# google/nerfactor

Measured on AMD Instinct MI355X. Metric: rays/sec (NeRF coarse+fine render, 64+128 samples/ray), higher is better.
Workload: dtype bf16

## Files before the change

### include/nfx.h

```cpp
#ifndef NFX_H_
#define NFX_H_

#include <stddef.h>
#include <stdint.h>

#ifdef __cplusplus
extern "C" {
#endif

#if defined(__GNUC__)
#define NFX_API __attribute__((visibility("default")))
#else
#define NFX_API
#endif

#define NFX_OK 0
#define NFX_EINVAL (-1)
#define NFX_EALIGN (-2)
#define NFX_EHIP (-3)
#define NFX_ENOSUP (-4)

#define NFX_PREC_BF16 0
#define NFX_PREC_FP32 1
#define NFX_PREC_FP32_NATIVE 2
// ... 187 lines not shown
#define NFX_LOSS_BLEND_A 1
#define NFX_LOSS_BLEND_B 2
#define NFX_LOSS_ACCUM_A 4
#define NFX_LOSS_ACCUM_B 8
typedef struct nfx_loss_term {
    const float *a, *b;
    float *ga, *gb;
    int d;
    float w;
    int kind;
    int flags;
} nfx_loss_term;
NFX_API int nfx_pair_loss_fwd(const nfx_loss_term *terms, int n_terms, const float *dev_alpha, float bg, int64_t n,
                      float *dev_loss, void *stream);
NFX_API int nfx_pair_loss_bwd(const nfx_loss_term *terms, int n_terms, const float *dev_alpha, float bg, int64_t n,
                      const float *dev_dloss, void *stream);


NFX_API int nfx_nerf_sigma_fwd(const float *dev_rayo, const float *dev_rayd, const float *dev_z, int64_t n_rays,
                       int n_samples, const void *dev_geom_blob, int prec, float *dev_sigma, void *stream);

NFX_API size_t nfx_nerf_geom_packed_bytes(int prec);
NFX_API int nfx_nerf_pack_geom_weights(const float *const kernels[12], const float *const biases[12], int prec,
                               void *blob, size_t blob_bytes);
NFX_API int nfx_nerf_sigma_grad(const float *dev_rayo, const float *dev_rayd, const float *dev_z, int64_t n_rays,
                        int n_samples, const void *dev_geom_blob, int prec, float *dev_normal_sigma,
                        void *stream);

NFX_API size_t nfx_nerf_sigma_grad_workspace_bytes(int64_t n_rays, int n_samples);
NFX_API int nfx_nerf_sigma_grad_rows(const float *dev_rayo, const float *dev_rayd, const float *dev_z, int64_t n_rays,
                             int n_samples, const void *dev_geom_blob, int prec, float *dev_normal_sigma,
                             void *dev_workspace, size_t workspace_bytes, void *stream);

NFX_API int nfx_nerf_refine_select(const float *dev_rgbs, const float *dev_z, const float *dev_rayd, int64_t n_rays,
                           int n_samples, float t_min, float a_lo, float a_hi, float sigma_margin, int dilate,
                           int *dev_list, int *dev_count, void *stream);
NFX_API int nfx_nerf_sigma_refine(const float *dev_rayo, const float *dev_rayd, const float *dev_z, int64_t n_rays,
                          int n_samples, const void *dev_geom_blob_fp32, const int *dev_list, const int *dev_count,
                          float *dev_rgbs, void *stream);

#define NFX_OCCGRID_MAX_RES 1024
#define NFX_OCCGRID_MAX_PROBES (1ll << 30)
NFX_API int nfx_nerf_sigma_fwd_list(const float *dev_rayo, const float *dev_rayd, const float *dev_z, int64_t n_rays,
                            int n_samples, const void *dev_geom_blob, int prec, const int *dev_list,
                            const int *dev_count, float *dev_sigma, void *stream);
NFX_API size_t nfx_occgrid_workspace_bytes(int64_t n_rays, int n_samples);
NFX_API int nfx_occgrid_select(const float *dev_rayo, const float *dev_rayd, const float *dev_z, int64_t n_rays,
                       int n_samples, const uint32_t *dev_bits, int res, const float *box, const float *bbox,
                       float *dev_sigma, void *dev_workspace, size_t workspace_bytes, void *stream);
NFX_API int nfx_occgrid_bake(const float *dev_probe_sigma, int res, int probes, float margin, int dilate,
                     uint32_t *dev_bits, uint32_t *dev_workspace, void *stream);


NFX_API int nfx_selftest_mfma_bf16(const float *dev_a, const float *dev_b, float *dev_d, void *stream);
NFX_API int nfx_mlp_generic_split_hilo(void *dev_blob, int d_in, int n_layers, const int *widths, const int *skip_input,
                                       int train, void *stream);
NFX_API size_t nfx_mlp_generic_packed_bytes(int d_in, int n_layers, const int *widths, const int *skip_input, int prec);
NFX_API int nfx_mlp_generic_pack(const float *const *kernels, const float *const *biases, int d_in, int n_layers,
                                 const int *widths, const int *skip_input, int prec, void *blob, size_t blob_bytes);
NFX_API int nfx_mlp_generic_fwd(const float *dev_x, int64_t n, int ld_x, int d_in, int n_layers, const int *widths,
                                const int *acts, const int *skip_input, const void *dev_blob, int prec, float *dev_y,
                                int ld_y, int col0, void *stream);
NFX_API size_t nfx_mlp_generic_train_packed_bytes(int d_in, int n_layers, const int *widths, const int *skip_input,
                                                  int prec);
NFX_API int nfx_mlp_generic_pack_train(const float *const *kernels, const float *const *biases, int d_in, int n_layers,
                                       const int *widths, const int *skip_input, int prec, void *blob,
// ... 21 lines not shown
```

### nerfactor_amd/_capi.py

```python
import ctypes
import os

import torch

_HERE = os.path.dirname(os.path.abspath(__file__))
LIB_PATH = os.path.join(_HERE, 'libnfx.so')
if os.environ.get('NFX_LIB_PATH'):
    LIB_PATH = os.environ['NFX_LIB_PATH']

PREC_BF16, PREC_FP32, PREC_FP32_NATIVE = 0, 1, 2
ACT_NONE, ACT_RELU, ACT_SIGMOID, ACT_SOFTPLUS = 0, 1, 2, 3
IN_XYZ, IN_XYZ_LDIR, IN_Z_RUSINK = 0, 1, 2

if not os.path.exists(LIB_PATH):
    raise ImportError(
        "%s not found: build it with `python -m nerfactor_amd.build` (or __graft_entry__.build()); "
        "nerfactor_amd has no fallback path." % LIB_PATH)

lib = ctypes.CDLL(LIB_PATH)

_p = ctypes.c_void_p
_i = ctypes.c_int
_i64 = ctypes.c_int64
_f = ctypes.c_float
# ... 35 lines not shown
    'nfx_composite_bwd': (_i, [_p, _p, _p, _p, _i64, _i, _i, _p, _p, _p]),
    'nfx_nerf_train_packed_bytes': (_sz, [_i]),
    'nfx_nerf_pack_train_weights': (_i, [_pp, _pp, _i, _p, _sz]),
    'nfx_nerf_bwd_workspace_bytes': (_sz, [_i64, _i]),
    'nfx_nerf_mlp_bwd': (_i, [_p, _p, _p, _i64, _i, _p, _i, _p, _p, _sz, _pp, _pp, _p]),
    'nfx_brdf_train_packed_bytes': (_sz, []),
    'nfx_brdf_pack_train_weights': (_i, [_pp, _pp, _i, _i, _p, _sz]),
    'nfx_brdf_spec_bwd_workspace_bytes': (_sz, [_i, _i64]),
    'nfx_brdf_spec_bwd': (_i, [_p, _p, _p, _p, _i, _p, _i, _p, _i, _i64, _p, _p, _p, _p, _sz, _p]),
    'nfx_brdf_spec_bwd_list_bytes': (_sz, [_i64, _i]),
    'nfx_brdf_spec_bwd_rows': (_i, [_p, _p, _p, _p, _i, _p, _i, _p, _i, _i64, _p, _p, _p, _p, _sz, _p, _sz, _p]),
    'nfx_brdf_rows_fwd': (_i, [_p, _i, _p, _i64, _i, _p, _i, _p, _p]),
    'nfx_brdf_rows_bwd_workspace_bytes': (_sz, [_i, _i64, _i]),
    'nfx_brdf_rows_bwd': (_i, [_p, _i, _p, _i64, _i, _p, _i, _p, _p, _sz, _p, _pp, _pp, _p]),
    'nfx_shade_bwd_workspace_bytes': (_sz, [_i]),
    'nfx_shade_bwd': (_i, [_p, _p, _p, _p, _p, _p, _f, _f, _p, _p, _p, _p, _i64, _i, _i, _p, _p, _p, _p, _p, _p,
                           _p, _p, _sz, _p]),
    'nfx_l2_normalize_rows': (_i, [_p, _p, _i64, _i, _f, _p]),
    'nfx_l2_normalize_rows_bwd': (_i, [_p, _p, _p, _i64, _i, _f, _p]),
    'nfx_light_smoothness': (_i, [_p, _i, _i, _f, _f, _p, _p, _p]),
    'nfx_pair_loss_fwd': (_i, [_p, _i, _p, _f, _i64, _p, _p]),
    'nfx_pair_loss_bwd': (_i, [_p, _i, _p, _f, _i64, _p, _p]),
    'nfx_pack_gather': (_i, [_p, _p, _i64, _p, _p]),
    'nfx_amsgrad_step': (_i, [_p, _p, _p, _p, _p, _i64, _f, _f, _f, _f, _i64, _p]),
    'nfx_amsgrad_step_size': (_f, [_f, _f, _f, _i64]),
    'nfx_amsgrad_step_dev': (_i, [_p, _p, _p, _p, _p, _i64, _p, _f, _f, _f, _p]),
    'nfx_nerf_sigma_fwd': (_i, [_p, _p, _p, _i64, _i, _p, _i, _p, _p]),
    'nfx_lvis_fwd_rows': (_i, [_p, _p, _i64, _f, _p, _i, _p, _i, _p, _sz, _p, _p, _p, _p]),
    'nfx_zero_rows': (_i, [_p, _p, _i64, _i, _p]),
    'nfx_shade_fwd_rows': (_i, [_p, _p, _p, _p, _p, _p, _f, _f, _p, _p, _p, _p, _p, _i64, _i, _i, _i, _p, _p]),
    'nfx_shade_olat_fwd_rows': (_i, [_p, _p, _p, _p, _p, _p, _f, _f, _p, _p, _p, _p, _f, _f, _i64, _i, _i, _p, _p, _p, _p]),
    'nfx_nerf_refine_select': (_i, [_p, _p, _p, _i64, _i, _f, _f, _f, _f, _i, _p, _p, _p]),
    'nfx_nerf_sigma_refine': (_i, [_p, _p, _p, _i64, _i, _p, _p, _p, _p, _p]),
    'nfx_nerf_sigma_fwd_list': (_i, [_p, _p, _p, _i64, _i, _p, _i, _p, _p, _p, _p]),
    'nfx_occgrid_workspace_bytes': (_sz, [_i64, _i]),
    'nfx_occgrid_select': (_i, [_p, _p, _p, _i64, _i, _p, _i, _p, _p, _p, _p, _sz, _p]),
    'nfx_occgrid_bake': (_i, [_p, _i, _i, _f, _i, _p, _p, _p]),
    'nfx_nerf_geom_packed_bytes': (_sz, [_i]),
    'nfx_nerf_pack_geom_weights': (_i, [_pp, _pp, _i, _p, _sz]),
    'nfx_nerf_sigma_grad': (_i, [_p, _p, _p, _i64, _i, _p, _i, _p, _p]),
    'nfx_nerf_sigma_grad_workspace_bytes': (_sz, [_i64, _i]),
    'nfx_nerf_sigma_grad_rows': (_i, [_p, _p, _p, _i64, _i, _p, _i, _p, _p, _sz, _p]),
    'nfx_selftest_mfma_bf16': (_i, [_p, _p, _p, _p]),
    'nfx_selftest_sincos': (_i, [_p, _i64, _i, _p, _p]),
    'nfx_selftest_tr16': (_i, [_p, _p, _p, _i, _p]),
    'nfx_mlp_generic_packed_bytes': (_sz, [_i, _i, _p, _p, _i]),
    'nfx_mlp_generic_pack': (_i, [_pp, _pp, _i, _i, _p, _p, _i, _p, _sz]),
    'nfx_mlp_generic_fwd': (_i, [_p, _i64, _i, _i, _i, _p, _p, _p, _p, _i, _p, _i, _i, _p]),
    'nfx_mlp_generic_train_packed_bytes': (_sz, [_i, _i, _p, _p, _i]),
    'nfx_mlp_generic_pack_train': (_i, [_pp, _pp, _i, _i, _p, _p, _i, _p, _sz]),
    'nfx_mlp_generic_bwd_workspace_bytes': (_sz, [_i64, _i, _i, _p, _p, _i]),
    'nfx_mlp_generic_split_hilo': (_i, [_p, _i, _i, _p, _p, _i, _p]),
    'nfx_brdf_rows_geom_fwd': (_i, [_p, _p, _p, _p, _i, _p, _i, _i64, _i, _p, _i, _p, _p]),
    'nfx_brdf_rows_geom_bwd': (_i, [_p, _p, _p, _i, _p, _i, _i64, _i, _p, _i, _p, _p, _p]),
    'nfx_embed_bwd': (_i, [_p, _i64, _i, _i, _p, _i, _i, _p, _p]),
    'nfx_mlp_generic_bwd': (_i, [_p, _i64, _i, _i, _i, _p, _p, _p, _p, _i, _p, _i, _i, _p, _i, _pp, _pp, _p, _sz, _p]),
    'nfx_embed': (_i, [_p, _p, _p, _i64, _i, _i, _i, _i, _p, _i, _i, _p]),
}

for _name, (_res, _args) in SIGNATURES.items():
    _fn = getattr(lib, _name)
    _fn.restype = _res
    _fn.argtypes = _args


class NfxError(RuntimeError):
# ... 59 lines not shown
```

### nerfactor_amd/csrc/capi_geom.cpp

```cpp
#include <hip/hip_runtime.h>
#include <math.h>
#include <string.h>

#include <vector>

#include "../../include/nfx.h"
#include "nerf_geom_layout.hpp"
#include "pack.hpp"

int nfx_fail(int code, const char* fmt, ...);
int nfx_hip_result(int e, const char* what);
extern "C" int nfx_option_int(const char* name, int dflt);

#define REQUIRE(cond, ...) \
    do {                   \
        if (!(cond)) return nfx_fail(NFX_EINVAL, __VA_ARGS__); \
    } while (0)
#define ALIGNED(p, a) ((((uintptr_t)(p)) & ((a)-1)) == 0)

extern "C" {
int nfx_launch_nerf_sigma_geo(const float*, const float*, const float*, long long, int, const void*, float*, int,
                              hipStream_t);
int nfx_launch_nerf_sigma_grad(const float*, const float*, const float*, long long, int, const void*, float*, int,
                               hipStream_t);
int nfx_launch_refine_select(const float*, const float*, const float*, long long, int, float, float, float, float, int, int*, int*,
                             hipStream_t);
int nfx_launch_nerf_sigma_v6(const float*, const float*, const float*, long long, int, const void*, float*, int, hipStream_t);
int nfx_launch_nerf_sigma_grad_list(const float*, const float*, const float*, long long, int, const void*, float*, const int*,
                                    const int*, int, hipStream_t);
int nfx_launch_nerf_sigma_grad_x3_list(const float*, const float*, const float*, long long, int, const void*, float*,
                                       const int*, const int*, int, hipStream_t);
int nfx_launch_select_density(const float*, long long, float*, void*, hipStream_t);
size_t nfx_nerf_bwd_list_bytes(long long n_pts);
int nfx_launch_nerf_sigma_x3_list(const float*, const float*, const float*, long long, int, const void*, float*, const int*,
                                  const int*, int, hipStream_t);
int nfx_launch_nerf_sigma_x3(const float*, const float*, const float*, long long, int, const void*, float*, int,
                             hipStream_t);
int nfx_launch_nerf_sigma_grad_x3(const float*, const float*, const float*, long long, int, const void*, float*, int,
                                  hipStream_t);
int nfx_launch_nerf_sigma_v6_list(const float*, const float*, const float*, long long, int, const void*, float*, const int*,
                                  const int*, int, hipStream_t);
int nfx_launch_nerf_sigma_x3_list_flat(const float*, const float*, const float*, long long, int, const void*, float*,
                                       const int*, const int*, int, hipStream_t);
size_t nfx_occgrid_list_bytes(long long n_pts);
int nfx_launch_occgrid_select(const float*, const float*, const float*, long long, int, const uint32_t*, int, const float*,
                              const float*, float*, void*, hipStream_t);
int nfx_launch_occgrid_bake(const float*, int, int, float, int, uint32_t*, uint32_t*, hipStream_t);

size_t nfx_nerf_geom_packed_bytes(int prec) {
    using namespace nfx::nerf;
    if (prec == NFX_PREC_BF16) return (size_t)kGeoBlobBytes;
    if (prec == NFX_PREC_FP32) return 2 * (size_t)kGeoWeightBytes + kGeoFloats * sizeof(float);
    return 0;
}
}

static int pack_geom_half(const float* const kernels[12], const float* const biases[12], uint8_t* w0, float* fl) {
    using namespace nfx;
    using namespace nfx::pack;
    std::vector<uint8_t> fwd(nfx_nerf_packed_bytes(NFX_PREC_BF16));
    int rc = nfx_nerf_pack_weights(kernels, biases, NFX_PREC_BF16, fwd.data(), fwd.size());
    if (rc) return rc;
    const size_t enc_bytes = (size_t)nerf::chunk_frag_offset(64) * 1024;
    memcpy(w0, fwd.data(), enc_bytes);
    memcpy(w0 + enc_bytes, fwd.data() + (size_t)nerf::chunk_frag_offset(72) * 1024, 16 * 1024);
    uint8_t* w = w0 + enc_bytes + 16 * 1024;
    std::vector<float> sink(256);
    const Seg hid256{kHidden, 256, 0, nullptr};
    auto hidden_t = [](const float* k) {
        std::vector<float> t((size_t)256 * 256);
        for (int r = 0; r < 256; ++r)
            for (int c = 0; c < 256; ++c) t[(size_t)c * 256 + r] = k[(size_t)r * 256 + c];
        return t;
    };
// ... 57 lines not shown
        }
        lo_ptr[i] = lo[i].data();
    }
    std::vector<float> sink(nerf::kGeoFloats);
    int rc = pack_geom_half(kernels, biases, w0, reinterpret_cast<float*>(w0 + 2 * (size_t)nerf::kGeoWeightBytes));
    if (rc) return rc;
    return pack_geom_half(lo_ptr, biases, w0 + nerf::kGeoWeightBytes, sink.data());
}

static int launch_sigma_bf16(const float* rayo, const float* rayd, const float* z, long long n_pts, int n_samples,
                             const void* blob, float* sigma, hipStream_t st) {
    const int blocks = nfx_option_int("nerf_blocks", 256);
    if (nfx_option_int("sigma_variant", 1) != 0)
        return nfx_launch_nerf_sigma_v6(rayo, rayd, z, n_pts, n_samples, blob, sigma, blocks, st);
    return nfx_launch_nerf_sigma_geo(rayo, rayd, z, n_pts, n_samples, blob, sigma, blocks, st);
}

int nfx_nerf_sigma_fwd(const float* rayo, const float* rayd, const float* z, int64_t n_rays, int n_samples,
                       const void* blob, int prec, float* sigma, void* stream) {
    REQUIRE(n_rays >= 0 && n_samples >= 1, "nfx_nerf_sigma_fwd: bad shape");
    REQUIRE(prec == NFX_PREC_BF16 || prec == NFX_PREC_FP32, "nfx_nerf_sigma_fwd: bad prec %d", prec);
    if (n_rays == 0) return NFX_OK;
    REQUIRE(rayo && rayd && z && blob && sigma, "nfx_nerf_sigma_fwd: null pointer");
    if (!ALIGNED(blob, 16)) return nfx_fail(NFX_EALIGN, "nfx_nerf_sigma_fwd: blob must be 16-byte aligned");
    if (prec == NFX_PREC_FP32)
        return nfx_hip_result(nfx_launch_nerf_sigma_x3(rayo, rayd, z, (long long)n_rays * n_samples, n_samples, blob,
                                                       sigma, nfx_option_int("nerf_blocks", 256), (hipStream_t)stream),
                              "nerf_sigma_fwd(fp32)");
    return nfx_hip_result(launch_sigma_bf16(rayo, rayd, z, (long long)n_rays * n_samples, n_samples, blob, sigma,
                                            (hipStream_t)stream),
                          "nerf_sigma_fwd");
}

int nfx_nerf_refine_select(const float* rgbs, const float* z, const float* rayd, int64_t n_rays, int n_samples,
                           float t_min, float a_lo, float a_hi, float sigma_margin, int dilate, int* list, int* count,
                           void* stream) {
    REQUIRE(n_rays >= 0 && n_samples >= 1 && n_samples <= 512, "nfx_nerf_refine_select: bad shape (1 <= S <= 512, got %d)", n_samples);
    REQUIRE(n_rays * (int64_t)n_samples < (int64_t)1 << 31, "nfx_nerf_refine_select: %lld samples do not fit int32 indices",
            (long long)(n_rays * n_samples));
    REQUIRE(dilate >= 0 && dilate <= 8, "nfx_nerf_refine_select: dilate = %d (0 .. 8)", dilate);
    REQUIRE(count, "nfx_nerf_refine_select: null count");
    if (n_rays > 0) REQUIRE(rgbs && z && rayd && list, "nfx_nerf_refine_select: null pointer");
    if (n_rays > 0 && !ALIGNED(rgbs, 16)) return nfx_fail(NFX_EALIGN, "nfx_nerf_refine_select: rgbs must be 16-byte aligned");
    return nfx_hip_result(nfx_launch_refine_select(rgbs, z, rayd, (long long)n_rays, n_samples, t_min, a_lo, a_hi, sigma_margin, dilate,
                                                   list, count, (hipStream_t)stream), "nerf_refine_select");
}

int nfx_nerf_sigma_refine(const float* rayo, const float* rayd, const float* z, int64_t n_rays, int n_samples,
                          const void* blob, const int* list, const int* count, float* rgbs, void* stream) {
    REQUIRE(n_rays >= 0 && n_samples >= 1, "nfx_nerf_sigma_refine: bad shape");
    if (n_rays == 0) return NFX_OK;
    REQUIRE(rayo && rayd && z && blob && list && count && rgbs, "nfx_nerf_sigma_refine: null pointer");
    if (!ALIGNED(blob, 16)) return nfx_fail(NFX_EALIGN, "nfx_nerf_sigma_refine: blob must be 16-byte aligned");
    return nfx_hip_result(nfx_launch_nerf_sigma_x3_list(rayo, rayd, z, (long long)n_rays * n_samples, n_samples, blob, rgbs,
                                                        list, count, nfx_option_int("nerf_blocks", 256),
                                                        (hipStream_t)stream), "nerf_sigma_refine");
}

int nfx_nerf_sigma_grad(const float* rayo, const float* rayd, const float* z, int64_t n_rays, int n_samples,
                        const void* geom_blob, int prec, float* normal_sigma, void* stream) {
    REQUIRE(n_rays >= 0 && n_samples >= 1, "nfx_nerf_sigma_grad: bad shape");
    REQUIRE(prec == NFX_PREC_BF16 || prec == NFX_PREC_FP32, "nfx_nerf_sigma_grad: bad prec %d", prec);
    if (n_rays == 0) return NFX_OK;
    REQUIRE(rayo && rayd && z && geom_blob && normal_sigma, "nfx_nerf_sigma_grad: null pointer");
    if (!ALIGNED(geom_blob, 16) || !ALIGNED(normal_sigma, 16))
        return nfx_fail(NFX_EALIGN, "nfx_nerf_sigma_grad: blob and output must be 16-byte aligned");
// ... 114 lines not shown
```

### nerfactor_amd/csrc/nerf_geom_x3.hip

```cpp
#include "feat_store.hpp"
#include "mlp_x3.hpp"
#include "nerf_geom_layout.hpp"

namespace nfx {
namespace geo3 {

using x3::Pair;
constexpr int kNW = x3::kNW;
constexpr int kRows = kNW * 32;
constexpr int kZeroTile = nerf::kGeoFloats;
constexpr int kLds = 2 * x3::kSlot + (nerf::kGeoFloats + 32) * 4;
constexpr int kNLD = 4;

template <int KS1, int KS2, int NL_SELF, int NL_NEXT, int KS1A, int KS2A>
__device__ __forceinline__ void fwd_layer(x3::Stream& st, int tid, const float* bias, const Pair (&b1)[KS1A],
                                          const Pair (&b2)[KS2A], Pair (&bout)[16], unsigned (&m)[4]) {
    static_for<0, 8>([&](auto T) {
        constexpr int t = decltype(T)::value;
        f32x16 acc;
        x3::tile<KS1, KS2, (t == 7 ? NL_NEXT : NL_SELF)>(st, tid, bias + 32 * t, b1, b2, acc);
        const unsigned bits = bwd::relu_bits16(acc);
        if constexpr (t & 1) m[t >> 1] |= bits << 16;
        else m[t >> 1] = bits;
        x3::acc_to_pair<true>(acc, bout[2 * t], bout[2 * t + 1]);
    });
}

__device__ __forceinline__ void put(Pair (&dst)[16], int t, int r, float v) {
    __bf16 a, b;
    x3::split(v, a, b);
    dst[2 * t + (r >> 3)].hi[r & 7] = a;
    dst[2 * t + (r >> 3)].lo[r & 7] = b;
}

__device__ __forceinline__ void dgrad(x3::Stream& st, int tid, const float* zero, const Pair (&dz)[16],
                                      const unsigned (&m)[4], Pair (&dout)[16]) {
    static_for<0, 8>([&](auto T) {
        constexpr int t = decltype(T)::value;
        f32x16 acc;
        x3::tile<16, 0, kNLD>(st, tid, zero, dz, dz, acc);
#pragma unroll
        for (int r = 0; r < 16; ++r) put(dout, t, r, bwd::mask_bit(m, t, r) ? acc[r] : 0.f);
    });
}

template <int NL_LAST>
__device__ __forceinline__ void input_grad(x3::Stream& st, int tid, const float* zero, const Pair (&dz)[16],
                                           f32x16 (&dpe)[2]) {
    static_for<0, 2>([&](auto T) {
        constexpr int t = decltype(T)::value;
        f32x16 acc;
        x3::tile<16, 0, (t == 1 ? NL_LAST : kNLD)>(st, tid, zero, dz, dz, acc);
#pragma unroll
        for (int r = 0; r < 16; ++r) dpe[t][r] += acc[r];
    });
}

template <bool GRAD>
__global__ __launch_bounds__(kNW * 64, 1) void nerf_sigma_x3_kernel(
    const float* __restrict__ rayo, const float* __restrict__ rayd, const float* __restrict__ zbuf, long long n_pts,
    int n_samples, const char* __restrict__ blob, float* __restrict__ out, const int* __restrict__ list,
    const int* __restrict__ count, int list_stride) {
    extern __shared__ __attribute__((aligned(16))) char smem[];
    using namespace nerf;
    if (list != nullptr) {
        n_pts = *count;
        if ((long long)blockIdx.x * kRows >= n_pts) return;
    }
    const int tid = threadIdx.x, lane = tid & 63, wave = tid >> 6, h = lane >> 5, p = lane & 31;
    float* fl = reinterpret_cast<float*>(smem + 2 * x3::kSlot);
    {
        const float* src = reinterpret_cast<const float*>(blob + 2 * (size_t)kGeoWeightBytes);
        for (int i = tid; i < kGeoFloats; i += kNW * 64) fl[i] = src[i];
        if (tid < 32) fl[kZeroTile + tid] = 0.f;
    }
    const float* zero = fl + kZeroTile;
    x3::Stream st;
    st.base = reinterpret_cast<const u32x4*>(blob);
    st.end = reinterpret_cast<const u32x4*>(blob + (GRAD ? (size_t)kGeoWeightBytes : (size_t)kGeoFwdFrags * kFragBytes));
    st.ghi = st.base;
    st.lo_off = kGeoWeightBytes / 16;
    st.ring = smem;
    x3::prologue<kNL0>(st, tid);
    const long long n_tiles = (n_pts + kRows - 1) / kRows;
    for (long long tile = blockIdx.x; tile < n_tiles; tile += gridDim.x) {
        const long long row = tile * kRows + wave * 32 + p;
        const bool valid = row < n_pts;
        long long mm = valid ? row : n_pts - 1;
        if (list != nullptr) mm = list[mm];
        float x[3];
        {
            const long long ray = mm / n_samples;
            const float zz = zbuf[mm];
#pragma unroll
            for (int k = 0; k < 3; ++k) x[k] = rayo[ray * 3 + k] + rayd[ray * 3 + k] * zz;
// ... 39 lines not shown
            input_grad<kNLD>(st, tid, zero, ha, dpe);
            dgrad(st, tid, zero, ha, mk[4], hb);
            dgrad(st, tid, zero, hb, mk[3], ha);
            dgrad(st, tid, zero, ha, mk[2], hb);
            dgrad(st, tid, zero, hb, mk[1], ha);
            dgrad(st, tid, zero, ha, mk[0], hb);
            input_grad<kNL0>(st, tid, zero, hb, dpe);
            float g[3] = {0.f, 0.f, 0.f};
#pragma unroll
            for (int q = 0; q < 32; ++q) {
                const float dq = dpe[q >> 4][q & 15];
                if (q < 30) {
                    const float freq = (float)(1 << (q / 3));
                    const float other = sin_shifted(x[q % 3] * freq, h ^ 1);
                    g[q % 3] += dq * freq * (h ? -other : other);
                } else if (q == 30) {
                    if (h) g[2] += dq; else g[0] += dq;
                } else {
                    if (!h) g[1] += dq;
                }
            }
#pragma unroll
            for (int k = 0; k < 3; ++k) g[k] += __shfl_xor(g[k], 32, 64);
            if (valid && h == 0) {
                const float on = sigma > 0.f ? 1.f : 0.f;
                const float gx = g[0] * on, gy = g[1] * on, gz = g[2] * on;
                const float inv = -1.0f / sqrtf(fmaxf(gx * gx + gy * gy + gz * gz, 1e-12f));
                reinterpret_cast<float4*>(out)[list != nullptr ? mm : row] = make_float4(gx * inv, gy * inv, gz * inv, sigma);
            }
        }
    }
}

template <bool GRAD>
static int launch(const float* rayo, const float* rayd, const float* z, long long n_pts, int n_samples,
                  const void* blob, float* out, int max_blocks, hipStream_t st, const int* list = nullptr,
                  const int* count = nullptr, int list_stride = 4) {
    if (n_pts <= 0) return 0;
    const long long tiles = (n_pts + kRows - 1) / kRows;
    const int grid = (int)(tiles < max_blocks ? tiles : max_blocks);
    auto k = nerf_sigma_x3_kernel<GRAD>;
    hipError_t e = hipFuncSetAttribute(reinterpret_cast<const void*>(k), hipFuncAttributeMaxDynamicSharedMemorySize, kLds);
    if (e != hipSuccess) return (int)e;
    hipLaunchKernelGGL(k, dim3(grid), dim3(kNW * 64), kLds, st, rayo, rayd, z, n_pts, n_samples, (const char*)blob, out,
                       list, count, list_stride);
    return (int)hipGetLastError();
}

}
}

extern "C" int nfx_launch_nerf_sigma_grad_x3(const float* rayo, const float* rayd, const float* z, long long n_pts,
                                             int n_samples, const void* blob, float* out, int max_blocks,
                                             hipStream_t st) {
    return nfx::geo3::launch<true>(rayo, rayd, z, n_pts, n_samples, blob, out, max_blocks, st);
}
extern "C" int nfx_launch_nerf_sigma_x3(const float* rayo, const float* rayd, const float* z, long long n_pts,
                                        int n_samples, const void* blob, float* out, int max_blocks, hipStream_t st) {
    return nfx::geo3::launch<false>(rayo, rayd, z, n_pts, n_samples, blob, out, max_blocks, st);
}
extern "C" int nfx_launch_nerf_sigma_grad_x3_list(const float* rayo, const float* rayd, const float* z, long long n_pts,
                                                  int n_samples, const void* blob, float* out, const int* list,
                                                  const int* count, int max_blocks, hipStream_t st) {
    return nfx::geo3::launch<true>(rayo, rayd, z, n_pts, n_samples, blob, out, max_blocks, st, list, count);
}
extern "C" int nfx_launch_nerf_sigma_x3_list(const float* rayo, const float* rayd, const float* z, long long n_pts,
                                             int n_samples, const void* blob, float* rgbs, const int* list,
                                             const int* count, int max_blocks, hipStream_t st) {
    return nfx::geo3::launch<false>(rayo, rayd, z, n_pts, n_samples, blob, rgbs, max_blocks, st, list, count);
}
extern "C" int nfx_launch_nerf_sigma_x3_list_flat(const float* rayo, const float* rayd, const float* z, long long n_pts,
                                                  int n_samples, const void* blob, float* out, const int* list,
                                                  const int* count, int max_blocks, hipStream_t st) {
    return nfx::geo3::launch<false>(rayo, rayd, z, n_pts, n_samples, blob, out, max_blocks, st, list, count, 1);
}
```

### nerfactor_amd/csrc/raymarch.hip

```cpp
#include "nfx_common.hpp"

namespace nfx {

__global__ void l2_normalize3_kernel(const float* __restrict__ in, float* __restrict__ out,
                                     long long n, float eps) {
    const long long i = (long long)blockIdx.x * blockDim.x + threadIdx.x;
    if (i >= n) return;
    const float x = in[3 * i], y = in[3 * i + 1], z = in[3 * i + 2];
    const float sq = x * x + y * y + z * z;
    const float inv = 1.0f / sqrtf(fmaxf(sq, eps));
    out[3 * i] = x * inv;
    out[3 * i + 1] = y * inv;
    out[3 * i + 2] = z * inv;
}

__device__ __forceinline__ float linspace01(int i, int n) { return (float)i * (1.0f / (float)(n - 1)); }

__device__ __forceinline__ float z_of_t(float t, float near, float far, int lin_in_disp) {
    if (lin_in_disp) return 1.0f / (1.0f / near * (1.0f - t) + 1.0f / far * t);
    return near * (1.0f - t) + far * t;
}

__global__ void gen_z_kernel(float near, float far, int n_samples, long long n_rays,
                             int lin_in_disp, const float* __restrict__ u, float* __restrict__ z) {
// ... 296 lines not shown
                                           dR2 * w * c2 * (1.f - c2), d_sg);
    }
}

__global__ __launch_bounds__(256) void sample_fine_kernel(
    const float* __restrict__ z, const float* __restrict__ weights, long long n_rays, int nc, int nf,
    const float* __restrict__ u, float* __restrict__ z_all) {
    extern __shared__ __attribute__((aligned(16))) char smem_raw[];
    float* smem = reinterpret_cast<float*>(smem_raw);
    const int lane = threadIdx.x & 63, wave = threadIdx.x >> 6;
    const int nb = nc - 2;
    const int ncdf = nc - 1;
    const int ntot = nc + nf;
    const int per_wave = 2 * ncdf + ntot;
    float* cdf = smem + wave * per_wave;
    float* mid = cdf + ncdf;
    float* zall = mid + ncdf;
    const long long ray = (long long)blockIdx.x * 4 + wave;
    const bool active = ray < n_rays;
    const long long rc = active ? ray : n_rays - 1;
    const float* zr = z + rc * nc;
    const float* wr = weights + rc * nc;

    for (int i = lane; i < nc; i += 64) zall[i] = zr[i];
    for (int i = lane; i < ncdf; i += 64) mid[i] = 0.5f * (zr[i + 1] + zr[i]);
    constexpr int kMaxSeg = 4;
    float wv[kMaxSeg];
#pragma unroll
    for (int k = 0; k < kMaxSeg; ++k) wv[k] = (64 * k + lane < nb) ? wr[1 + 64 * k + lane] : 0.f;
    float denom = 0.f;
#pragma unroll
    for (int k = 0; k < kMaxSeg; ++k) {
        const int cnt = nb - 64 * k < 64 ? nb - 64 * k : 64;
        for (int i = 0; i < cnt; ++i) denom += __shfl(wv[k], i, 64);
    }
    denom += 1e-5f;
    float pdf[kMaxSeg], cv[kMaxSeg];
#pragma unroll
    for (int k = 0; k < kMaxSeg; ++k) {
        pdf[k] = wv[k] / denom;
        cv[k] = 0.f;
    }
    float acc = 0.f;
#pragma unroll
    for (int k = 0; k < kMaxSeg; ++k) {
        const int cnt = nb - 64 * k < 64 ? nb - 64 * k : 64;
        for (int i = 0; i < cnt; ++i) {
            acc += __shfl(pdf[k], i, 64);
            if (lane == i) cv[k] = acc;
        }
    }
    if (lane == 0) cdf[0] = 0.f;
#pragma unroll
    for (int k = 0; k < kMaxSeg; ++k)
        if (64 * k + lane < nb) cdf[1 + 64 * k + lane] = cv[k];
    __syncthreads();
    for (int i = lane; i < nf; i += 64) {
        const float uu = u ? u[rc * nf + i] : linspace01(i, nf);
        int lo = 0, hi = ncdf;
        while (lo < hi) {
            const int m = (lo + hi) >> 1;
            if (cdf[m] <= uu) lo = m + 1; else hi = m;
        }
        const int ind = lo;
        const int below = ind - 1 > 0 ? ind - 1 : 0;
        const int above = ind < ncdf - 1 ? ind : ncdf - 1;
        const float cb = cdf[below], ca = cdf[above];
        float den = ca - cb;
        den = den < 1e-5f ? 1.0f : den;
        const float t = (uu - cb) / den;
        const float vb = mid[below], va = mid[above];
        zall[nc + i] = vb + t * (va - vb);
    }
    __syncthreads();
    if (u == nullptr) {
        const float* zc = zall;
        const float* zf = zall + nc;
        for (int i = lane; i < ntot; i += 64) {
            const float v = zall[i];
            int lo = 0, hi, rank;
            if (i < nc) {
// ... 173 lines not shown
```

### nerfactor_amd/ops.py

```python
import ctypes
import os

import numpy as np
import torch

from . import _capi
from ._capi import PREC_BF16, PREC_FP32, PREC_FP32_NATIVE, check, lib

_PREC = {'bf16': PREC_BF16, 'fp32': PREC_FP32, 'fp32_native': PREC_FP32_NATIVE, PREC_BF16: PREC_BF16, PREC_FP32: PREC_FP32,
         PREC_FP32_NATIVE: PREC_FP32_NATIVE}
_ACT = {None: 0, 'none': 0, 'relu': 1, 'sigmoid': 2, 'softplus': 3}


def _ptr(t):
    return None if t is None else ctypes.c_void_p(t.data_ptr())


def _stream():
    return ctypes.c_void_p(torch.cuda.current_stream().cuda_stream)


def _dev(t, name, shape=None):
    if t is None:
        return None
# ... 778 lines not shown
            first = ws_bytes // 4 - nerf_bwd_list_words((hi - lo) * s)[3]
            NERF_BWD_STATS.append((ws.view(torch.int32)[first:first + 1].clone(), (hi - lo) * s))
    return ws


def pack_nerf_geom_weights(kernels, biases, prec='bf16'):
    if len(kernels) != 12 or len(biases) != 12:
        raise _capi.NfxError("pack_nerf_geom_weights: need 12 kernels and 12 biases")
    return _pack(lib.nfx_nerf_geom_packed_bytes, lib.nfx_nerf_pack_geom_weights, kernels, biases, (_PREC[prec],))


def _ray_args(rayo, rayd, z, blob):
    rayo = _dev(rayo, 'rayo', (None, 3))
    n = rayo.shape[0]
    rayd = _dev(rayd, 'rayd', (n, 3))
    z = _dev(z, 'z', (n, None))
    if not blob.is_cuda or blob.dtype != torch.uint8:
        raise _capi.NfxError("blob must be a CUDA uint8 tensor")
    return rayo, rayd, z, n, z.shape[1]


def nerf_sigma_fwd(rayo, rayd, z, blob, prec='bf16'):
    rayo, rayd, z, n, s = _ray_args(rayo, rayd, z, blob)
    out = torch.empty((n, s), dtype=torch.float32, device=z.device)
    check(lib.nfx_nerf_sigma_fwd(_ptr(rayo), _ptr(rayd), _ptr(z), n, s, _ptr(blob), _PREC[prec], _ptr(out),
                                 _stream()), 'nfx_nerf_sigma_fwd')
    return out


def nerf_refine_last_sample(rayo, rayd, z, rgbs, geom_blob_fp32):
    n, s = z.shape
    if n == 0 or s < 2:
        return rgbs
    sig = nerf_sigma_fwd(rayo, rayd, z[:, -1:].contiguous(), geom_blob_fp32, 'fp32')
    rgbs[:, -1, 3] = sig[:, 0]
    return rgbs


REFINE_T_MIN, REFINE_A_LO, REFINE_A_HI, REFINE_DILATE = 1e-3, 1e-3, 0.999, 0
REFINE_MARGIN_FACTOR = 2.


def nerf_refine_coarse(rayo, rayd, z, rgbs, geom_blob_fp32, t_min=REFINE_T_MIN, a_lo=REFINE_A_LO, a_hi=REFINE_A_HI,
                       dilate=REFINE_DILATE, sigma_margin=0., want_count=False):
    rayo, rayd, z, n, s = _ray_args(rayo, rayd, z, geom_blob_fp32)
    if not (isinstance(rgbs, torch.Tensor) and rgbs.is_contiguous()):
        raise _capi.NfxError("nerf_refine_coarse: rgbs is updated in place and must be contiguous")
    rgbs = _dev(rgbs, 'rgbs', (n, s, 4))
    count = torch.empty(1, dtype=torch.int32, device=z.device)
    if n == 0 or s < 2:
        count.zero_()
        return (rgbs, count) if want_count else rgbs
    lst = torch.empty(n * s, dtype=torch.int32, device=z.device)
    check(lib.nfx_nerf_refine_select(_ptr(rgbs), _ptr(z), _ptr(rayd), n, s, t_min, a_lo, a_hi, sigma_margin, dilate, _ptr(lst), _ptr(count),
                                     _stream()), 'nfx_nerf_refine_select')
    check(lib.nfx_nerf_sigma_refine(_ptr(rayo), _ptr(rayd), _ptr(z), n, s, _ptr(geom_blob_fp32), _ptr(lst), _ptr(count),
                                    _ptr(rgbs), _stream()), 'nfx_nerf_sigma_refine')
    return (rgbs, count) if want_count else rgbs


def nerf_coarse_error(rayo, rayd, z, rgbs, geom_blob_fp32, max_rays=4096, q=0.999, geom_blob_bf16=None):
    n = min(int(z.shape[0]), max_rays)
    if n == 0 or z.shape[1] < 2:
        return 0., 0.
    step = max(1, int(z.shape[0]) // n)
    pick = slice(0, n * step, step)
    o, d, zz = rayo[pick].contiguous(), rayd[pick].contiguous(), z[pick].contiguous()
    s32 = nerf_sigma_fwd(o, d, zz, geom_blob_fp32, 'fp32')
# ... 240 lines not shown
```

Baseline: 4.513 million.

## Add LDS-DMA ring-pipelined sigma kernel and fused last-sample refine column path

Specializes the non-gradient sigma kernel to stream weight chunks into a 3-slot LDS ring via direct global-to-LDS DMA, prefetching two chunks ahead so weight loads overlap the MFMA work. It also adds a column mode that evaluates sigma for the last sample of each ray and writes it straight into the rgbs tensor. This replaces the Python slice/contiguous copy, the separate kernel output and the scatter. The sample_fine CDF loops now use readlane instead of shfl. In exchange the code is more complex, relies on hand-tuned vmcnt waits, and uses more LDS.

```diff
diff --git a/include/nfx.h b/include/nfx.h
--- a/include/nfx.h
+++ b/include/nfx.h
@@ -243,6 +243,8 @@
                              int n_samples, const void *dev_geom_blob, int prec, float *dev_normal_sigma,
                              void *dev_workspace, size_t workspace_bytes, void *stream);
 
+NFX_API int nfx_nerf_refine_last_sample(const float *dev_rayo, const float *dev_rayd, const float *dev_z, int64_t n_rays,
+                                int n_samples, const void *dev_geom_blob_fp32, float *dev_rgbs, void *stream);
 NFX_API int nfx_nerf_refine_select(const float *dev_rgbs, const float *dev_z, const float *dev_rayd, int64_t n_rays,
                            int n_samples, float t_min, float a_lo, float a_hi, float sigma_margin, int dilate,
                            int *dev_list, int *dev_count, void *stream);
diff --git a/nerfactor_amd/_capi.py b/nerfactor_amd/_capi.py
--- a/nerfactor_amd/_capi.py
+++ b/nerfactor_amd/_capi.py
@@ -91,6 +91,7 @@
     'nfx_shade_olat_fwd_rows': (_i, [_p, _p, _p, _p, _p, _p, _f, _f, _p, _p, _p, _p, _f, _f, _i64, _i, _i, _p, _p, _p, _p]),
     'nfx_nerf_refine_select': (_i, [_p, _p, _p, _i64, _i, _f, _f, _f, _f, _i, _p, _p, _p]),
     'nfx_nerf_sigma_refine': (_i, [_p, _p, _p, _i64, _i, _p, _p, _p, _p, _p]),
+    'nfx_nerf_refine_last_sample': (_i, [_p, _p, _p, _i64, _i, _p, _p, _p]),
     'nfx_nerf_sigma_fwd_list': (_i, [_p, _p, _p, _i64, _i, _p, _i, _p, _p, _p, _p]),
     'nfx_occgrid_workspace_bytes': (_sz, [_i64, _i]),
     'nfx_occgrid_select': (_i, [_p, _p, _p, _i64, _i, _p, _i, _p, _p, _p, _p, _sz, _p]),
diff --git a/nerfactor_amd/csrc/capi_geom.cpp b/nerfactor_amd/csrc/capi_geom.cpp
--- a/nerfactor_amd/csrc/capi_geom.cpp
+++ b/nerfactor_amd/csrc/capi_geom.cpp
@@ -40,6 +40,8 @@
                                   hipStream_t);
 int nfx_launch_nerf_sigma_v6_list(const float*, const float*, const float*, long long, int, const void*, float*, const int*,
                                   const int*, int, hipStream_t);
+int nfx_launch_nerf_sigma_x3_column(const float*, const float*, const float*, long long, int, int, const void*, float*, int,
+                                    hipStream_t);
 int nfx_launch_nerf_sigma_x3_list_flat(const float*, const float*, const float*, long long, int, const void*, float*,
                                        const int*, const int*, int, hipStream_t);
 size_t nfx_occgrid_list_bytes(long long n_pts);
@@ -163,6 +165,17 @@
                           "nerf_sigma_fwd");
 }
 
+int nfx_nerf_refine_last_sample(const float* rayo, const float* rayd, const float* z, int64_t n_rays, int n_samples,
+                                const void* blob, float* rgbs, void* stream) {
+    REQUIRE(n_rays >= 0 && n_samples >= 1, "nfx_nerf_refine_last_sample: bad shape");
+    if (n_rays == 0) return NFX_OK;
+    REQUIRE(rayo && rayd && z && blob && rgbs, "nfx_nerf_refine_last_sample: null pointer");
+    if (!ALIGNED(blob, 16)) return nfx_fail(NFX_EALIGN, "nfx_nerf_refine_last_sample: blob must be 16-byte aligned");
+    return nfx_hip_result(nfx_launch_nerf_sigma_x3_column(rayo, rayd, z, (long long)n_rays, n_samples, n_samples - 1, blob,
+                                                          rgbs, nfx_option_int("nerf_blocks", 256), (hipStream_t)stream),
+                          "nerf_refine_last_sample");
+}
+
 int nfx_nerf_refine_select(const float* rgbs, const float* z, const float* rayd, int64_t n_rays, int n_samples,
                            float t_min, float a_lo, float a_hi, float sigma_margin, int dilate, int* list, int* count,
                            void* stream) {
diff --git a/nerfactor_amd/csrc/nerf_geom_x3.hip b/nerfactor_amd/csrc/nerf_geom_x3.hip
--- a/nerfactor_amd/csrc/nerf_geom_x3.hip
+++ b/nerfactor_amd/csrc/nerf_geom_x3.hip
@@ -1,4 +1,5 @@
 #include "feat_store.hpp"
+#include "lds_dma.hpp"
 #include "mlp_x3.hpp"
 #include "nerf_geom_layout.hpp"
 
@@ -60,7 +61,7 @@
 __global__ __launch_bounds__(kNW * 64, 1) void nerf_sigma_x3_kernel(
     const float* __restrict__ rayo, const float* __restrict__ rayd, const float* __restrict__ zbuf, long long n_pts,
     int n_samples, const char* __restrict__ blob, float* __restrict__ out, const int* __restrict__ list,
-    const int* __restrict__ count, int list_stride) {
+    const int* __restrict__ count, int list_stride, int ) {
     extern __shared__ __attribute__((aligned(16))) char smem[];
     using namespace nerf;
     if (list != nullptr) {
@@ -166,18 +167,171 @@
     }
 }
 
+namespace dma {
+
+constexpr int kChunks = 65;
+constexpr int kRing = 3;
+constexpr int kLds = kRing * x3::kSlot + nerf::kGeoFloats * 4;
+static_assert(kLds <= 160 * 1024, "LDS budget");
+constexpr int frags(int c) { return nerf::chunk_frags(c % kChunks); }
+static_assert(nerf::chunk_frag_offset(kChunks) == nerf::kGeoFwdFrags, "the density stream is chunks 0 .. 64");
+static_assert(frags(0) == 4 * nerf::kNL0 && frags(8) == 4 * nerf::kNLH && frags(40) == 4 * nerf::kNL5 &&
+                  frags(64) == 4 * nerf::kNLH && 4 * nerf::kNL5 <= kSlotFrags,
+              "chunk sizes of the register-staged stream");
+
+struct Ring {
+    const char* blob;
+    char* smem;
+    unsigned lds;
+    unsigned wave;
+    unsigned lane_off;
+    int cur;
+};
+
+template <int C>
+__device__ __forceinline__ void fetch(const Ring& r, int slot) {
+    constexpr int c = C % kChunks;
+    constexpr int nl = frags(c) / 4;
+    const char* g = r.blob + ((size_t)nerf::chunk_frag_offset(c) + r.wave * nl) * kFragBytes;
+    const unsigned d = r.lds + slot * x3::kSlot + r.wave * nl * kFragBytes;
+#pragma unroll
+    for (int half = 0; half < 2; ++half) {
+        const char* gh = g + (half ? (size_t)nerf::kGeoWeightBytes : 0);
+        const unsigned dh = d + half * kSlotBytes;
+        if constexpr (nl <= 4) {
+            lds_dma_pieces<nl>(r.lane_off, gh, dh);
+        } else {
+            lds_dma_pieces<3>(r.lane_off, gh, dh);
+            lds_dma_pieces<nl - 3>(r.lane_off, gh + 3 * kFragBytes, dh + 3 * kFragBytes);
+        }
+    }
+}
+
+template <int N>
+__device__ __forceinline__ void wait_vm() {
+    asm volatile("s_waitcnt vmcnt(%0)" ::"n"(N) : "memory");
+}
+
+__device__ __forceinline__ int slot_after(int s, int k) {
+    s += k;
+    return s >= kRing ? s - kRing : s;
+}
+
+template <int C, int KS1, int KS2, int KS1A, int KS2A, typename E>
+__device__ __forceinline__ void tile(Ring& r, int lane, const float* bias_tile, const Pair (&b1)[KS1A],
+                                     const Pair (&b2)[KS2A], f32x16& acc, E&& epi) {
+    fetch<C + 2>(r, slot_after(r.cur, 2));
+    {
+        f32x16 a1[1];
+        bias_init<1>(bias_tile, lane >> 5, a1);
+        acc = a1[0];
+    }
+    const char* fh = r.smem + r.cur * x3::kSlot + lane * 16;
+    const char* fl = fh + kSlotBytes;
+    static_for<0, KS1 + KS2>([&](auto S) {
+        constexpr int s = decltype(S)::value;
+        const bf16x8 ah = *reinterpret_cast<const bf16x8*>(fh + s * kFragBytes);
+        const bf16x8 al = *reinterpret_cast<const bf16x8*>(fl + s * kFragBytes);
+        const Pair& b = s < KS1 ? b1[s < KS1 ? s : 0] : b2[s >= KS1 ? s - KS1 : 0];
+        acc = __builtin_amdgcn_mfma_f32_32x32x16_bf16(al, b.hi, acc, 0, 0, 0);
+        acc = __builtin_amdgcn_mfma_f32_32x32x16_bf16(ah, b.lo, acc, 0, 0, 0);
+        acc = __builtin_amdgcn_mfma_f32_32x32x16_bf16(ah, b.hi, acc, 0, 0, 0);
+    });
+    epi();
+    wait_vm<2 * (frags(C + 2) / 4)>();
+    __syncthreads();
+    r.cur = slot_after(r.cur, 1);
+}
+
+template <int C0, int KS1, int KS2, int KS1A, int KS2A>
+__device__ __forceinline__ void layer(Ring& r, int lane, const float* bias, const Pair (&b1)[KS1A],
+                                      const Pair (&b2)[KS2A], Pair (&bout)[16]) {
+    f32x16 acc[2];
+    static_for<0, 8>([&](auto T) {
+        constexpr int t = decltype(T)::value;
+        tile<C0 + t, KS1, KS2>(r, lane, bias + 32 * t, b1, b2, acc[t & 1], [&] {
+            if constexpr (t > 0) x3::acc_to_pair<true>(acc[(t - 1) & 1], bout[2 * (t - 1)], bout[2 * (t - 1) + 1]);
+        });
+    });
+    x3::acc_to_pair<true>(acc[1], bout[14], bout[15]);
+}
+
+}
+
+template <>
+__global__ __launch_bounds__(kNW * 64, 1) void nerf_sigma_x3_kernel<false>(
+    const float* __restrict__ rayo, const float* __restrict__ rayd, const float* __restrict__ zbuf, long long n_pts,
+    int n_samples, const char* __restrict__ blob, float* __restrict__ out, const int* __restrict__ list,
+    const int* __restrict__ count, int out_stride, int col) {
+    extern __shared__ __attribute__((aligned(16))) char smem[];
+    using namespace nerf;
+    using namespace dma;
+    if (list != nullptr) {
+        n_pts = *count;
+        if ((long long)blockIdx.x * kRows >= n_pts) return;
+    }
+    const int tid = threadIdx.x, lane = tid & 63, wave = tid >> 6, h = lane >> 5, p = lane & 31;
+    float* fl = reinterpret_cast<float*>(smem + kRing * x3::kSlot);
+    {
+        const float* src = reinterpret_cast<const float*>(blob + 2 * (size_t)kGeoWeightBytes);
+        for (int i = tid; i < kGeoFloats; i += kNW * 64) fl[i] = src[i];
+    }
+    typedef __attribute__((address_space(3))) char lds_char;
+    Ring r{blob, smem, (unsigned)__builtin_amdgcn_readfirstlane((unsigned)(uintptr_t)(lds_char*)smem),
+           (unsigned)__builtin_amdgcn_readfirstlane(tid >> 6), (unsigned)lane * 16u, 0};
+    fetch<0>(r, 0);
+    fetch<1>(r, 1);
+    wait_vm<2 * (frags(1) / 4)>();
+    __syncthreads();
+    const long long n_tiles = (n_pts + kRows - 1) / kRows;
+    for (long long tile_i = blockIdx.x; tile_i < n_tiles; tile_i += gridDim.x) {
+        const long long row = tile_i * kRows + wave * 32 + p;
+        const bool valid = row < n_pts;
+        long long mm = valid ? row : n_pts - 1;
+        if (list != nullptr) mm = list[mm];
+        else if (col >= 0) mm = mm * n_samples + col;
+        float x[3];
+        {
+            const long long ray = mm / n_samples;
+            const float zz = zbuf[mm];
+#pragma unroll
+            for (int k = 0; k < 3; ++k) x[k] = rayo[ray * 3 + k] + rayd[ray * 3 + k] * zz;
+        }
+        Pair pe[4];
+        x3::posenc_pair<10>(x, h, pe);
+        Pair ha[16], hb[16];
+        layer<0, 4, 0>(r, lane, fl + 256 * 0, pe, pe, ha);
+        layer<8, 16, 0>(r, lane, fl + 256 * 1, ha, pe, hb);
+        layer<16, 16, 0>(r, lane, fl + 256 * 2, hb, pe, ha);
+        layer<24, 16, 0>(r, lane, fl + 256 * 3, ha, pe, hb);
+        layer<32, 16, 0>(r, lane, fl + 256 * 4, hb, pe, ha);
+        layer<40, 16, 4>(r, lane, fl + 256 * 5, ha, pe, hb);
+        layer<48, 16, 0>(r, lane, fl + 256 * 6, hb, pe, ha);
+        layer<56, 16, 0>(r, lane, fl + 256 * 7, ha, pe, hb);
+        f32x16 acc;
+        tile<64, 16, 0>(r, lane, fl + kGeoBiasSig, hb, pe, acc, [] {});
+        const float sigma = acc[0];
+        if (valid && h == 0) {
+            if (list != nullptr || col >= 0) out[out_stride * (mm + 1) - 1] = sigma;
+            else out[row] = sigma;
+        }
+    }
+    wait_vm<0>();
+}
+
 template <bool GRAD>
 static int launch(const float* rayo, const float* rayd, const float* z, long long n_pts, int n_samples,
                   const void* blob, float* out, int max_blocks, hipStream_t st, const int* list = nullptr,
-                  const int* count = nullptr, int list_stride = 4) {
+                  const int* count = nullptr, int list_stride = 4, int col = -1) {
     if (n_pts <= 0) return 0;
     const long long tiles = (n_pts + kRows - 1) / kRows;
     const int grid = (int)(tiles < max_blocks ? tiles : max_blocks);
+    constexpr int lds = GRAD ? kLds : dma::kLds;
     auto k = nerf_sigma_x3_kernel<GRAD>;
-    hipError_t e = hipFuncSetAttribute(reinterpret_cast<const void*>(k), hipFuncAttributeMaxDynamicSharedMemorySize, kLds);
+    hipError_t e = hipFuncSetAttribute(reinterpret_cast<const void*>(k), hipFuncAttributeMaxDynamicSharedMemorySize, lds);
     if (e != hipSuccess) return (int)e;
-    hipLaunchKernelGGL(k, dim3(grid), dim3(kNW * 64), kLds, st, rayo, rayd, z, n_pts, n_samples, (const char*)blob, out,
-                       list, count, list_stride);
+    hipLaunchKernelGGL(k, dim3(grid), dim3(kNW * 64), lds, st, rayo, rayd, z, n_pts, n_samples, (const char*)blob, out,
+                       list, count, list_stride, col);
     return (int)hipGetLastError();
 }
 
@@ -208,3 +362,8 @@
                                                   const int* count, int max_blocks, hipStream_t st) {
     return nfx::geo3::launch<false>(rayo, rayd, z, n_pts, n_samples, blob, out, max_blocks, st, list, count, 1);
 }
+extern "C" int nfx_launch_nerf_sigma_x3_column(const float* rayo, const float* rayd, const float* z, long long n_rays,
+                                               int n_samples, int col, const void* blob, float* rgbs, int max_blocks,
+                                               hipStream_t st) {
+    return nfx::geo3::launch<false>(rayo, rayd, z, n_rays, n_samples, blob, rgbs, max_blocks, st, nullptr, nullptr, 4, col);
+}
diff --git a/nerfactor_amd/csrc/raymarch.hip b/nerfactor_amd/csrc/raymarch.hip
--- a/nerfactor_amd/csrc/raymarch.hip
+++ b/nerfactor_amd/csrc/raymarch.hip
@@ -352,7 +352,7 @@
 #pragma unroll
     for (int k = 0; k < kMaxSeg; ++k) {
         const int cnt = nb - 64 * k < 64 ? nb - 64 * k : 64;
-        for (int i = 0; i < cnt; ++i) denom += __shfl(wv[k], i, 64);
+        for (int i = 0; i < cnt; ++i) denom += __int_as_float(__builtin_amdgcn_readlane(__float_as_int(wv[k]), i));
     }
     denom += 1e-5f;
     float pdf[kMaxSeg], cv[kMaxSeg];
@@ -366,7 +366,7 @@
     for (int k = 0; k < kMaxSeg; ++k) {
         const int cnt = nb - 64 * k < 64 ? nb - 64 * k : 64;
         for (int i = 0; i < cnt; ++i) {
-            acc += __shfl(pdf[k], i, 64);
+            acc += __int_as_float(__builtin_amdgcn_readlane(__float_as_int(pdf[k]), i));
             if (lane == i) cv[k] = acc;
         }
     }
diff --git a/nerfactor_amd/ops.py b/nerfactor_amd/ops.py
--- a/nerfactor_amd/ops.py
+++ b/nerfactor_amd/ops.py
@@ -834,8 +834,12 @@
     n, s = z.shape
     if n == 0 or s < 2:
         return rgbs
-    sig = nerf_sigma_fwd(rayo, rayd, z[:, -1:].contiguous(), geom_blob_fp32, 'fp32')
-    rgbs[:, -1, 3] = sig[:, 0]
+    rayo, rayd, z, n, s = _ray_args(rayo, rayd, z, geom_blob_fp32)
+    dst = _dev(rgbs, 'rgbs', (n, s, 4))
+    check(lib.nfx_nerf_refine_last_sample(_ptr(rayo), _ptr(rayd), _ptr(z), n, s, _ptr(geom_blob_fp32), _ptr(dst), _stream()),
+          'nfx_nerf_refine_last_sample')
+    if dst is not rgbs:
+        rgbs.copy_(dst)
     return rgbs
 
 
```

Result: no change. 4.556 million, median of 6 (+0.9%).
